# tkkim-robot/safe_control

Hardware: AMD Instinct MI355X
Metric: QP solves/sec (batched agents) (higher is better)
Workload: dtype f64; 1 GPU; 4096-agent batch DynamicUnicycle2D CBF-QP, 8 obstacles each (BASELINE configs[1]); agents_per_gpu=4096, obstacles=8, storage=f32, arithmetic=f64, launch=hipGraph

## Files before the change

### safe_control_amd/csrc/cbf_qp_kernel.hpp

```cpp
#pragma once
#include <hip/hip_runtime.h>

#include <utility>

#include <cstdlib>

#include "sc_qp2.hpp"
#include "sc_group.hpp"

namespace sc {

#ifndef SC_COOP_MAX_AGENTS
#define SC_COOP_MAX_AGENTS 32768
#endif

static inline long long sc_coop_max_agents() {
    static const long long v = [] { const char* e = getenv("SC_COOP_MAX_AGENTS"); return e ? atoll(e) : (long long)SC_COOP_MAX_AGENTS; }();
    return v;
}
static inline bool sc_two_pass() {
    static const bool v = [] { const char* e = getenv("SC_CBFQP_TWO_PASS"); return !(e && e[0] == '0'); }();
    return v;
}
static inline bool sc_force_lds_kernel() {
    static const bool v = [] { const char* e = getenv("SC_FORCE_LDS_KERNEL"); return e && e[0] == '1'; }();
    return v;
}

using as1_void = const __attribute__((address_space(1))) void;
using as3_void = __attribute__((address_space(3))) void;

template <typename TIO, int MODEL>
struct StateRow { TIO v[MODEL == SC_MODEL_QUAD2D ? 5 : 4]; };

template <typename TIO, int MODEL>
__device__ __forceinline__ StateRow<TIO, MODEL> load_state(const TIO* __restrict__ X, long long agent) {
    StateRow<TIO, MODEL> s;
    if constexpr (MODEL == SC_MODEL_QUAD2D) {
        const TIO* r = X + agent * 6;
#pragma unroll
        for (int i = 0; i < 5; ++i) s.v[i] = r[i];
    } else {
        const TIO* r = X + agent * 4;
#pragma unroll
        for (int i = 0; i < 4; ++i) s.v[i] = r[i];
    }
    return s;
}

template <typename TIO, typename TC, int MODEL>
__device__ __forceinline__ Agent<TC> to_agent(const StateRow<TIO, MODEL>& s) {
    if constexpr (MODEL == SC_MODEL_QUAD2D) return make_agent_m<TC, MODEL>(TC(s.v[0]), TC(s.v[1]), TC(s.v[2]), TC(s.v[3]), TC(s.v[4]));
    else return make_agent_m<TC, MODEL>(TC(s.v[0]), TC(s.v[1]), TC(s.v[2]), TC(s.v[3]));
}

template <typename TIO, typename TC, int MODEL>
__device__ __forceinline__ Agent<TC> load_agent(const TIO* __restrict__ X, long long agent) {
    return to_agent<TIO, TC, MODEL>(load_state<TIO, MODEL>(X, agent));
}

template <typename T>
__device__ __forceinline__ void fetch_arg_now(const T& v) { asm volatile("" ::"s"(v)); }

template <typename TIO> struct vec2;
template <> struct vec2<float> { using type = float2; };
template <> struct vec2<double> { using type = double2; };

__device__ __forceinline__ void wave_dma16(const unsigned char* __restrict__ src, unsigned char* lds,
                                           unsigned bytes, int lane) {
    const unsigned n16 = bytes >> 4;
    for (unsigned base = 0; base < n16; base += 64) {
        const unsigned idx = base + lane;
        if (idx < n16) {
            __builtin_amdgcn_global_load_lds((as1_void*)(src + (size_t)idx * 16),
                                             (as3_void*)(lds + (size_t)base * 16), 16, 0, 0);
        }
    }
}

template <typename TIO> struct vec4io;
template <> struct vec4io<float> { using type = float4; static constexpr int N = 4; };
template <> struct vec4io<double> { using type = double2; static constexpr int N = 2; };

#define SC_STATUS_PENDING (-1)
template <typename TIO, typename TC, int KMAX, int MODEL, int PASS = 0>
__global__ __launch_bounds__(256) void cbfqp_reg_kernel(const TIO* __restrict__ obs, const TIO* __restrict__ X,
                                                        const TIO* __restrict__ u_ref, const int* __restrict__ n_obs,
                                                        const long long B, const int K, const int obs_shared,
                                                        TIO* __restrict__ u_out, int* __restrict__ status_out,
                                                        TIO* __restrict__ h_out, const CbfConsts<TC> k) {
    const long long agent = (long long)blockIdx.x * blockDim.x + threadIdx.x;
    const bool active = agent < B;
    const long long ag_i = active ? agent : 0;
    using V2 = typename vec2<TIO>::type;
    using V4 = typename vec4io<TIO>::type;
    constexpr int VN = vec4io<TIO>::N;
    if constexpr (PASS == 2) {
        const bool pending = active && status_out[ag_i] == SC_STATUS_PENDING;
        if (__builtin_amdgcn_ballot_w64(pending) == 0ull) return;
    }

    TIO flat[KMAX * 7];
    const TIO* src = obs + (obs_shared ? 0 : (size_t)ag_i * K * 7);
    if (K == KMAX && ((KMAX * 7) % VN == 0) && ((reinterpret_cast<uintptr_t>(obs) & 15u) == 0) &&
        ((KMAX * 7 * sizeof(TIO)) % 16 == 0)) {
        const V4* s4 = reinterpret_cast<const V4*>(src);
#pragma unroll
        for (int e = 0; e < KMAX * 7 / VN; ++e) {
            const V4 q = s4[e];
            if constexpr (VN == 4) {
                flat[e * 4 + 0] = q.x; flat[e * 4 + 1] = q.y; flat[e * 4 + 2] = q.z; flat[e * 4 + 3] = q.w;
            } else {
                flat[e * 2 + 0] = q.x; flat[e * 2 + 1] = q.y;
            }
        }
    } else {
#pragma unroll
        for (int r = 0; r < KMAX; ++r) {
#pragma unroll
            for (int f = 0; f < 7; ++f) flat[r * 7 + f] = (r < K) ? src[r * 7 + f] : TIO(0);
        }
    }
    const V2 ur = reinterpret_cast<const V2*>(u_ref)[ag_i];
    const StateRow<TIO, MODEL> xs = load_state<TIO, MODEL>(X, ag_i);
    int nk = K;
    if (n_obs) nk = n_obs[ag_i];
    nk = nk < 0 ? 0 : (nk > K ? K : nk);
    if constexpr (PASS == 1) {
        bool other = false;
#pragma unroll
        for (int r = 0; r < KMAX; ++r) other |= (r < nk) && (flat[r * 7 + 6] != TIO(0));
        if (__builtin_amdgcn_ballot_w64(other && active) != 0ull) {
            if (active) status_out[agent] = SC_STATUS_PENDING;
            return;
        }
    }
    const TC ur0 = TC(ur.x), ur1 = TC(ur.y);
    const Agent<TC> ag = to_agent<TIO, TC, MODEL>(xs);

    TC n0[KMAX], n1[KMAX], c[KMAX];
    TIO hv[KMAX];
    bool bad_obs = false;
    TC poison = TC(0);
#pragma unroll
    for (int r = 0; r < KMAX; ++r) {
        TC o[7];
#pragma unroll
        for (int f = 0; f < 7; ++f) o[f] = TC(flat[r * 7 + f]);
        TC h, a0, a1, cc;
        const bool ok = cbf_row<TC, MODEL, true, PASS == 1>(ag, o, k, a0, a1, cc, h);
        const bool used = r < nk;
        bad_obs |= used && !ok;
        a0 = used ? a0 : TC(0); a1 = used ? a1 : TC(0); cc = used ? cc : TC(0);
        normalise_row(a0, a1, cc, poison);
        n0[r] = a0; n1[r] = a1; c[r] = cc;
        hv[r] = used ? TIO(h) : TIO(0);
    }

    TC u0, u1;
    int st = qp2_solve<TC, KMAX>(n0, n1, c, K, ur0, ur1, poison, k, u0, u1);
    if (bad_obs) st = SC_STATUS_BAD_OBSTACLE;
    if (st != SC_STATUS_OPTIMAL) { u0 = num<TC>::nan(); u1 = num<TC>::nan(); }
    if (active) {
        V2 uo; uo.x = TIO(u0); uo.y = TIO(u1);
        reinterpret_cast<V2*>(u_out)[agent] = uo;
        status_out[agent] = st;
        if (h_out) {
            TIO* hp = h_out + agent * K;
            if (K == KMAX && (KMAX % VN == 0) && ((reinterpret_cast<uintptr_t>(h_out) & 15u) == 0)) {
                V4* h4 = reinterpret_cast<V4*>(hp);
#pragma unroll
                for (int e = 0; e < KMAX / VN; ++e) {
                    V4 q;
                    if constexpr (VN == 4) { q.x = hv[e * 4]; q.y = hv[e * 4 + 1]; q.z = hv[e * 4 + 2]; q.w = hv[e * 4 + 3]; }
                    else { q.x = hv[e * 2]; q.y = hv[e * 2 + 1]; }
                    h4[e] = q;
                }
            } else {
#pragma unroll
                for (int r = 0; r < KMAX; ++r) if (r < K) hp[r] = hv[r];
            }
        }
    }
}

template <typename TIO, typename TC, int G, int MODEL>
#ifndef SC_COOP_WAVES
#define SC_COOP_WAVES 1
#endif
__global__ __launch_bounds__(64 * SC_COOP_WAVES) void cbfqp_coop_kernel(const TIO* __restrict__ obs, const TIO* __restrict__ X,
                                                        const TIO* __restrict__ u_ref, const int* __restrict__ n_obs,
                                                        const long long B, const int K, const int obs_shared,
                                                        TIO* __restrict__ u_out, int* __restrict__ status_out,
                                                        TIO* __restrict__ h_out, const CbfConsts<TC> k) {
#ifdef SC_EXP_EMPTY
    return;
#endif
    constexpr int APW = 64 / G;
    const int lane = threadIdx.x & 63;
    const int sub = lane & (G - 1);
    const long long agent = ((long long)blockIdx.x * SC_COOP_WAVES + (threadIdx.x >> 6)) * APW + lane / G;
    const bool active = agent < B;
    const long long ag_i = active ? agent : 0;
    using V2 = typename vec2<TIO>::type;
#ifdef SC_EXP_ARGS
    if (active && sub == 0)
        status_out[agent] = (int)((reinterpret_cast<uintptr_t>(obs) ^ reinterpret_cast<uintptr_t>(X) ^ reinterpret_cast<uintptr_t>(u_ref) ^
                                   reinterpret_cast<uintptr_t>(n_obs) ^ reinterpret_cast<uintptr_t>(u_out) ^ reinterpret_cast<uintptr_t>(h_out)) >> 4) + K + obs_shared;
    return;
#endif

    TIO orow[7];
    const bool has_row = sub < K;
    const TIO* src = obs + (obs_shared ? 0 : (size_t)ag_i * K * 7) + (has_row ? sub * 7 : 0);
#pragma unroll
    for (int f = 0; f < 7; ++f) orow[f] = src[f];
    const V2 ur = reinterpret_cast<const V2*>(u_ref)[ag_i];
    const StateRow<TIO, MODEL> xs = load_state<TIO, MODEL>(X, ag_i);
    int nk = K;
    if (n_obs) nk = n_obs[ag_i];
    nk = nk < 0 ? 0 : (nk > K ? K : nk);
    fetch_arg_now(status_out); fetch_arg_now(h_out);
    fetch_arg_now(k.R); fetch_arg_now(k.g1); fetch_arg_now(k.g2);
    fetch_arg_now(k.lo0); fetch_arg_now(k.hi0); fetch_arg_now(k.lo1); fetch_arg_now(k.hi1); fetch_arg_now(k.hard);
#ifdef SC_EXP_LOADS
    if (active) {
        if (sub == 0) {
            V2 uo; uo.x = ur.x + xs.v[0] + xs.v[1]; uo.y = ur.y + xs.v[2] + xs.v[3];
            reinterpret_cast<V2*>(u_out)[agent] = uo;
            status_out[agent] = nk;
        }
        if (h_out && has_row) h_out[agent * K + sub] = orow[0] + orow[1] + orow[2] + orow[3] + orow[4] + orow[5] + orow[6];
    }
    return;
#endif
    const TC ur0 = TC(ur.x), ur1 = TC(ur.y);
    const Agent<TC> ag = to_agent<TIO, TC, MODEL>(xs);

    TC o[7];
#pragma unroll
    for (int f = 0; f < 7; ++f) o[f] = TC(orow[f]);
    TC h, a0, a1, cc;
#ifndef SC_EXP_NOROW
    const bool ok = cbf_row<TC, MODEL, false>(ag, o, k, a0, a1, cc, h);
#else
    const bool ok = true; a0 = o[0] - ag.x; a1 = o[1] - ag.y; cc = o[2]; h = o[3];
#endif
    const bool used = sub < nk;
    const bool bad_mine = used && !ok;
    a0 = used ? a0 : TC(0); a1 = used ? a1 : TC(0); cc = used ? cc : TC(0);
    if (active && h_out && has_row) h_out[agent * K + sub] = used ? TIO(h) : TIO(0);
    TC poison = TC(0);
    normalise_row(a0, a1, cc, poison);

    QpState<TC> S;
    qp_begin(S, ur0, ur1, k);
#ifndef SC_EXP_NOWALK
#ifndef SC_COOP_OLD_WALK
    if constexpr (G == 8) coop_solve_all8<TC>(S, K, sub, lane, a0, a1, cc, k);
    else if constexpr (G == 16) coop_solve_all16<TC>(S, K, sub, lane, a0, a1, cc, k);
    else
#endif
    coop_walk_violated<TC, G>(S, K, sub, lane, a0, a1, cc, k);
#endif
    qp_finish_box(S, k);
    TC worst = qp_row_margin(num<TC>::inf(), a0, a1, cc, S.u0, S.u1, poison);
    const bool nan_mine = !(poison == poison);
    worst = nan_mine ? -num<TC>::inf() : worst;
    if constexpr (G == 8) worst = min8_raw(worst);
    else if constexpr (G == 16) worst = min16_raw(worst);
    else worst = group_min<TC, G>(worst);
    const unsigned long long bad_mask = __builtin_amdgcn_ballot_w64(bad_mine);
    const bool bad_any = ((bad_mask >> (lane & ~(G - 1))) & (G == 64 ? ~0ull : ((1ull << G) - 1ull))) != 0ull;
    int st = qp_status(S, worst, TC(0), k);
    if (bad_any) st = SC_STATUS_BAD_OBSTACLE;
    TC u0 = S.u0, u1 = S.u1;
    if (st != SC_STATUS_OPTIMAL) { u0 = num<TC>::nan(); u1 = num<TC>::nan(); }
    if (active) {
        if (sub == 0) {
            V2 uo; uo.x = TIO(u0); uo.y = TIO(u1);
            reinterpret_cast<V2*>(u_out)[agent] = uo;
            status_out[agent] = st;
        }
    }
}

template <typename TIO, typename TC, int G, int MODEL>
static hipError_t launch_coop(const sc_cbfqp_params& p, long long B, int K, const void* X, const void* u_ref,
                              const void* obs, const int* n_obs, void* u_out, int* status, void* h_out,
                              hipStream_t stream) {
    constexpr int APW = 64 / G;
    const unsigned nblk = (unsigned)((B + APW * SC_COOP_WAVES - 1) / (APW * SC_COOP_WAVES));
    const CbfConsts<TC> k = make_consts<TC>(p);
    hipLaunchKernelGGL((cbfqp_coop_kernel<TIO, TC, G, MODEL>), dim3(nblk), dim3(64 * SC_COOP_WAVES), 0, stream,
                       (const TIO*)obs, (const TIO*)X, (const TIO*)u_ref, n_obs, B, K, (int)p.obs_shared,
                       (TIO*)u_out, status, (TIO*)h_out, k);
    return hipGetLastError();
}

template <typename TIO, typename TC, int KMAX, int MODEL>
__global__ __launch_bounds__(64) void cbfqp_kernel(const TIO* __restrict__ obs, const TIO* __restrict__ X,
                                                   const TIO* __restrict__ u_ref, const int* __restrict__ n_obs,
                                                   const long long B, const int K, const int obs_shared,
                                                   TIO* __restrict__ u_out, int* __restrict__ status_out,
                                                   TIO* __restrict__ h_out, const CbfConsts<TC> k) {
    extern __shared__ __attribute__((aligned(16))) unsigned char smem[];
    TIO* lobs = reinterpret_cast<TIO*>(smem);

    const int lane = threadIdx.x;
    const long long first = (long long)blockIdx.x * 64;
    const long long agent = first + lane;
    const int nag = (int)((B - first) < 64 ? (B - first) : 64);
    const bool active = lane < nag;
    const int row_elems = K * 7;

    if (obs_shared) {
        for (int e = lane; e < row_elems; e += 64) lobs[e] = obs[e];
    } else {
        const TIO* src = obs + (size_t)first * row_elems;
        const unsigned bytes = (unsigned)nag * row_elems * sizeof(TIO);
        if ((bytes & 15u) == 0 && ((reinterpret_cast<uintptr_t>(src) & 15u) == 0)) {
            wave_dma16(reinterpret_cast<const unsigned char*>(src), smem, bytes, lane);
        } else {
            const int total = nag * row_elems;
            for (int e = lane; e < total; e += 64) lobs[e] = src[e];
        }
    }

    using V2 = typename vec2<TIO>::type;
    const long long ag_i = active ? agent : 0;
    const V2 ur = reinterpret_cast<const V2*>(u_ref)[ag_i];
    const StateRow<TIO, MODEL> xs = load_state<TIO, MODEL>(X, ag_i);
    int nk = K;
    if (n_obs) nk = n_obs[ag_i];
    nk = !active ? K : (nk < 0 ? 0 : (nk > K ? K : nk));
    const TC ur0 = active ? TC(ur.x) : TC(0), ur1 = active ? TC(ur.y) : TC(0);
    const Agent<TC> ag = to_agent<TIO, TC, MODEL>(xs);

    asm volatile("s_waitcnt vmcnt(0)" ::: "memory");
    __syncthreads();

    const size_t stage_bytes = ((obs_shared ? (size_t)row_elems : (size_t)64 * row_elems) * sizeof(TIO) + 15) & ~(size_t)15;
    TC* rows = reinterpret_cast<TC*>(smem + stage_bytes);
    TIO* hl = reinterpret_cast<TIO*>(rows + (size_t)K * 3 * 64);
    const TIO* mine = lobs + (obs_shared ? 0 : lane * row_elems);
    int period = 32;
    while (((K * (32 / period)) & 31) != 0 && period > 1) period >>= 1;
    const int rot = obs_shared ? 0 : (lane / period) % K;
    bool bad_obs = false;
    TC poison = TC(0);
#pragma nounroll
    for (int r = 0; r < K; ++r) {
        int ro = r + rot;
        ro = ro >= K ? ro - K : ro;
        TC o[7];
#pragma unroll
        for (int f = 0; f < 7; ++f) o[f] = TC(mine[ro * 7 + f]);
        TC h, a0, a1, cc;
        const bool ok = cbf_row<TC, MODEL>(ag, o, k, a0, a1, cc, h);
        const bool used = ro < nk;
        bad_obs |= used && !ok;
        a0 = used ? a0 : TC(0); a1 = used ? a1 : TC(0); cc = used ? cc : TC(0);
        normalise_row(a0, a1, cc, poison);
        rows[(ro * 3 + 0) * 64 + lane] = a0;
        rows[(ro * 3 + 1) * 64 + lane] = a1;
        rows[(ro * 3 + 2) * 64 + lane] = cc;
        if constexpr (KMAX > 0) {
            hl[ro * 64 + lane] = used ? TIO(h) : TIO(0);
        } else {
            if (active && h_out) h_out[agent * K + ro] = used ? TIO(h) : TIO(0);
        }
    }

    TC u0, u1;
    int st;
    if constexpr (KMAX > 0) {
        TC n0[KMAX], n1[KMAX], c[KMAX];
#pragma unroll
        for (int j = 0; j < KMAX; ++j) {
            const bool in = j < K;
            n0[j] = in ? rows[(j * 3 + 0) * 64 + lane] : TC(0);
            n1[j] = in ? rows[(j * 3 + 1) * 64 + lane] : TC(0);
            c[j] = in ? rows[(j * 3 + 2) * 64 + lane] : TC(0);
        }
        st = qp2_solve<TC, KMAX>(n0, n1, c, K, ur0, ur1, poison, k, u0, u1);
    } else {
        st = qp2_solve_lds<TC>(rows, lane, K, ur0, ur1, poison, k, u0, u1);
    }

    if (bad_obs) st = SC_STATUS_BAD_OBSTACLE;
    if (st != SC_STATUS_OPTIMAL) { u0 = num<TC>::nan(); u1 = num<TC>::nan(); }

    if (active) {
        V2 uo; uo.x = TIO(u0); uo.y = TIO(u1);
        reinterpret_cast<V2*>(u_out)[agent] = uo;
        status_out[agent] = st;
        if constexpr (KMAX > 0) {
            if (h_out) {
                TIO* hp = h_out + agent * K;
                if (K == KMAX) {
                    TIO hv[KMAX];
#pragma unroll
                    for (int r = 0; r < KMAX; ++r) hv[r] = hl[r * 64 + lane];
#pragma unroll
                    for (int r = 0; r < KMAX; ++r) hp[r] = hv[r];
                } else {
                    for (int r = 0; r < K; ++r) hp[r] = hl[r * 64 + lane];
                }
            }
        }
    }
}

template <typename TIO, typename TC, int KMAX, int MODEL>
static hipError_t launch_one(const sc_cbfqp_params& p, long long B, int K, const void* X, const void* u_ref,
                             const void* obs, const int* n_obs, void* u_out, int* status, void* h_out,
                             hipStream_t stream) {
    if constexpr (KMAX > 0) {
        if (B <= sc_coop_max_agents())
            return launch_coop<TIO, TC, 8, MODEL>(p, B, K, X, u_ref, obs, n_obs, u_out, status, h_out, stream);
        const unsigned threads = 256;
        const unsigned nblk = (unsigned)((B + threads - 1) / threads);
        const CbfConsts<TC> k = make_consts<TC>(p);
        if constexpr (MODEL == SC_MODEL_DYNAMIC_UNICYCLE2D && sizeof(TC) == 8) {
            if (sc_two_pass() && B >= (1 << 18)) {
                hipLaunchKernelGGL((cbfqp_reg_kernel<TIO, TC, KMAX, MODEL, 1>), dim3(nblk), dim3(threads), 0, stream,
                                   (const TIO*)obs, (const TIO*)X, (const TIO*)u_ref, n_obs, B, K, (int)p.obs_shared,
                                   (TIO*)u_out, status, (TIO*)h_out, k);
                hipError_t e = hipGetLastError();
                if (e != hipSuccess) return e;
                hipLaunchKernelGGL((cbfqp_reg_kernel<TIO, TC, KMAX, MODEL, 2>), dim3(nblk), dim3(threads), 0, stream,
                                   (const TIO*)obs, (const TIO*)X, (const TIO*)u_ref, n_obs, B, K, (int)p.obs_shared,
                                   (TIO*)u_out, status, (TIO*)h_out, k);
                return hipGetLastError();
            }
        }
        hipLaunchKernelGGL((cbfqp_reg_kernel<TIO, TC, KMAX, MODEL>), dim3(nblk), dim3(threads), 0, stream,
                           (const TIO*)obs, (const TIO*)X, (const TIO*)u_ref, n_obs, B, K, (int)p.obs_shared,
                           (TIO*)u_out, status, (TIO*)h_out, k);
        return hipGetLastError();
    } else {
    if (!sc_force_lds_kernel()) {
        if (K <= 16) return launch_coop<TIO, TC, 16, MODEL>(p, B, K, X, u_ref, obs, n_obs, u_out, status, h_out, stream);
        return launch_coop<TIO, TC, 32, MODEL>(p, B, K, X, u_ref, obs, n_obs, u_out, status, h_out, stream);
    }
    const unsigned blocks = (unsigned)((B + 63) / 64);
    const CbfConsts<TC> k = make_consts<TC>(p);
    size_t lds = (p.obs_shared ? (size_t)K * 7 : (size_t)64 * K * 7) * sizeof(TIO);
    lds = ((lds + 15) & ~(size_t)15) + (size_t)K * 3 * 64 * sizeof(TC) + (KMAX > 0 ? (size_t)K * 64 * sizeof(TIO) : 0);
    auto kern = cbfqp_kernel<TIO, TC, KMAX, MODEL>;
    if (lds > 64 * 1024) {
        static bool raised = false;
        if (!raised) {
            hipError_t e = hipFuncSetAttribute(reinterpret_cast<const void*>(kern),
                                               hipFuncAttributeMaxDynamicSharedMemorySize, 160 * 1024);
            if (e != hipSuccess) return e;
            raised = true;
        }
    }
    hipLaunchKernelGGL(kern, dim3(blocks), dim3(64), lds, stream,
                       (const TIO*)obs, (const TIO*)X, (const TIO*)u_ref, n_obs, B, K, (int)p.obs_shared,
                       (TIO*)u_out, status, (TIO*)h_out, k);
    return hipGetLastError();
    }
}

template <typename TIO, typename TC, int MODEL>
static hipError_t launch_k(const sc_cbfqp_params& p, long long B, int K, const void* X, const void* u_ref,
                           const void* obs, const int* n_obs, void* u_out, int* status, void* h_out,
                           hipStream_t stream) {
#define SC_K(KM) return launch_one<TIO, TC, KM, MODEL>(p, B, K, X, u_ref, obs, n_obs, u_out, status, h_out, stream)
    if (K <= 4) SC_K(4);
    if (K <= 8) SC_K(8);
    SC_K(0);
#undef SC_K
}

template <typename TIO, typename TC>
static hipError_t launch_model(const sc_cbfqp_params& p, long long B, int K, const void* X, const void* u_ref,
                               const void* obs, const int* n_obs, void* u_out, int* status, void* h_out,
                               hipStream_t stream) {
    switch (p.model_id) {
        case SC_MODEL_DYNAMIC_UNICYCLE2D:
            return launch_k<TIO, TC, SC_MODEL_DYNAMIC_UNICYCLE2D>(p, B, K, X, u_ref, obs, n_obs, u_out, status, h_out, stream);
        case SC_MODEL_KINEMATIC_BICYCLE2D:
            return launch_k<TIO, TC, SC_MODEL_KINEMATIC_BICYCLE2D>(p, B, K, X, u_ref, obs, n_obs, u_out, status, h_out, stream);
        case SC_MODEL_KINEMATIC_BICYCLE2D_C3BF:
            return launch_k<TIO, TC, SC_MODEL_KINEMATIC_BICYCLE2D_C3BF>(p, B, K, X, u_ref, obs, n_obs, u_out, status, h_out, stream);
        case SC_MODEL_SINGLE_INTEGRATOR2D:
            return launch_k<TIO, TC, SC_MODEL_SINGLE_INTEGRATOR2D>(p, B, K, X, u_ref, obs, n_obs, u_out, status, h_out, stream);
        case SC_MODEL_DOUBLE_INTEGRATOR2D:
            return launch_k<TIO, TC, SC_MODEL_DOUBLE_INTEGRATOR2D>(p, B, K, X, u_ref, obs, n_obs, u_out, status, h_out, stream);
        case SC_MODEL_QUAD2D:
            return launch_k<TIO, TC, SC_MODEL_QUAD2D>(p, B, K, X, u_ref, obs, n_obs, u_out, status, h_out, stream);
        case SC_MODEL_UNICYCLE2D:
            return launch_k<TIO, TC, SC_MODEL_UNICYCLE2D>(p, B, K, X, u_ref, obs, n_obs, u_out, status, h_out, stream);
        default:
            return launch_k<TIO, TC, SC_MODEL_KINEMATIC_BICYCLE2D_DPCBF>(p, B, K, X, u_ref, obs, n_obs, u_out, status, h_out, stream);
    }
}

}
```

### safe_control_amd/csrc/sc_group.hpp

```cpp
#pragma once
#include <hip/hip_runtime.h>

#include <utility>

#include "sc_qp2.hpp"

namespace sc {

template <int CTRL>
__device__ __forceinline__ float dpp_mov(float v) {
    return __int_as_float(__builtin_amdgcn_update_dpp(0, __float_as_int(v), CTRL, 0xf, 0xf, true));
}
template <int CTRL>
__device__ __forceinline__ double dpp_mov(double v) {
    const int lo = __builtin_amdgcn_update_dpp(0, __double2loint(v), CTRL, 0xf, 0xf, true);
    const int hi = __builtin_amdgcn_update_dpp(0, __double2hiint(v), CTRL, 0xf, 0xf, true);
    return __hiloint2double(hi, lo);
}
template <typename T, int G, int I>
__device__ __forceinline__ T group_bcast(T v, int sub) {
    if constexpr (G == 8) {
        const T q = dpp_mov<(I & 3) * 0x55>(v);
        const T m = dpp_mov<0x141>(q);
        return ((sub >> 2) == (I >> 2)) ? q : m;
    } else {
        return __shfl(v, I, G);
    }
}
template <typename T, int G>
__device__ __forceinline__ T group_max(T v) {
    if constexpr (G == 8) {
        v = fmax_(v, dpp_mov<0xB1>(v)); v = fmax_(v, dpp_mov<0x4E>(v)); v = fmax_(v, dpp_mov<0x141>(v));
    } else {
#pragma unroll
        for (int o = 1; o < G; o <<= 1) v = fmax_(v, __shfl_xor(v, o));
    }
    return v;
}
template <typename T, int G>
__device__ __forceinline__ T group_min(T v) {
    if constexpr (G == 8) {
        v = fmin_(v, dpp_mov<0xB1>(v)); v = fmin_(v, dpp_mov<0x4E>(v)); v = fmin_(v, dpp_mov<0x141>(v));
    } else {
#pragma unroll
        for (int o = 1; o < G; o <<= 1) v = fmin_(v, __shfl_xor(v, o));
    }
    return v;
}

template <typename TC, int G, int I>
__device__ __forceinline__ void coop_step(QpState<TC>& S, int K, int sub, TC a0, TC a1, TC cc, const CbfConsts<TC>& k) {
    if (I >= K) return;
    const TC bi0 = group_bcast<TC, G, I>(a0, sub), bi1 = group_bcast<TC, G, I>(a1, sub), bic = group_bcast<TC, G, I>(cc, sub);
    LineQP<TC> L;
    const bool viol = qp_row_violated(S, bi0, bi1, bic, L, k);
    if (__builtin_amdgcn_ballot_w64(viol) == 0) return;
    clip_box(L, k);
    if (sub < I) clip_row(L, a0, a1, cc);
    L.lo = group_max<TC, G>(L.lo);
    L.hi = group_min<TC, G>(L.hi);
    qp_row_commit(S, L, viol);
}
template <typename TC, int G, int... Is>
__device__ __forceinline__ void coop_walk(QpState<TC>& S, int K, int sub, TC a0, TC a1, TC cc, const CbfConsts<TC>& k,
                                          std::integer_sequence<int, Is...>) {
    (coop_step<TC, G, Is>(S, K, sub, a0, a1, cc, k), ...);
}

template <typename TC, int G>
__device__ __forceinline__ void coop_walk_violated(QpState<TC>& S, int K, int sub, int lane, TC a0, TC a1, TC cc,
                                                   const CbfConsts<TC>& k) {
    const int gbase = lane & ~(G - 1);
    const unsigned long long grp = (G == 64 ? ~0ull : ((1ull << G) - 1ull)) << gbase;
    const bool testable = (sub < K) && !((a0 == TC(0)) && (a1 == TC(0)));
    int last = -1;
#ifndef SC_EXP_MAXIT
#define SC_EXP_MAXIT G
#endif
    for (int it = 0; it < SC_EXP_MAXIT; ++it) {
        const TC s = a0 * S.u0 + (a1 * S.u1 + cc);
        const bool v = testable && (sub > last) && (s < TC(0));
        const unsigned long long m = __builtin_amdgcn_ballot_w64(v);
        if (m == 0ull) break;
        const unsigned long long mg = m & grp;
        const bool has = mg != 0ull;
        const int istar = has ? (__builtin_ctzll(mg) - gbase) : 0;
        const TC bi0 = __shfl(a0, istar, G), bi1 = __shfl(a1, istar, G), bic = __shfl(cc, istar, G);
        LineQP<TC> L;
        const bool viol = qp_row_violated(S, bi0, bi1, bic, L, k) && has;
        clip_box(L, k);
        if (sub < istar) clip_row(L, a0, a1, cc);
        L.lo = group_max<TC, G>(L.lo);
        L.hi = group_min<TC, G>(L.hi);
        qp_row_commit(S, L, viol);
        last = has ? istar : K;
    }
}

template <typename T, int X>
__device__ __forceinline__ T group_xor8(T v, T mirrored) {
    if constexpr (X == 1) return dpp_mov<0xB1>(v);
    else if constexpr (X == 2) return dpp_mov<0x4E>(v);
    else if constexpr (X == 3) return dpp_mov<0x1B>(v);
    else if constexpr (X == 4) return dpp_mov<0x1B>(mirrored);
    else if constexpr (X == 5) return dpp_mov<0x4E>(mirrored);
    else if constexpr (X == 6) return dpp_mov<0xB1>(mirrored);
    else return mirrored;
}
__device__ __forceinline__ float min_raw(float a, float b) { float r; asm("v_min_f32 %0, %1, %2" : "=v"(r) : "v"(a), "v"(b)); return r; }
__device__ __forceinline__ float max_raw(float a, float b) { float r; asm("v_max_f32 %0, %1, %2" : "=v"(r) : "v"(a), "v"(b)); return r; }
__device__ __forceinline__ double min_raw(double a, double b) { double r; asm("v_min_f64 %0, %1, %2" : "=v"(r) : "v"(a), "v"(b)); return r; }
__device__ __forceinline__ double max_raw(double a, double b) { double r; asm("v_max_f64 %0, %1, %2" : "=v"(r) : "v"(a), "v"(b)); return r; }
__device__ __forceinline__ float max_neg_raw(float a, float b) { float r; asm("v_max_f32 %0, %1, -%2" : "=v"(r) : "v"(a), "v"(b)); return r; }
__device__ __forceinline__ double max_neg_raw(double a, double b) { double r; asm("v_max_f64 %0, %1, -%2" : "=v"(r) : "v"(a), "v"(b)); return r; }
__device__ __forceinline__ float max_abs_one_raw(float a) { float r; asm("v_max_f32 %0, |%1|, 1.0" : "=v"(r) : "v"(a)); return r; }
__device__ __forceinline__ double max_abs_one_raw(double a) { double r; asm("v_max_f64 %0, |%1|, 1.0" : "=v"(r) : "v"(a)); return r; }
__device__ __forceinline__ float keep_or_nan(bool keep, float v) { return keep ? v : __int_as_float(0x7fc00000); }
__device__ __forceinline__ double keep_or_nan(bool keep, double v) {
    return __hiloint2double(keep ? __double2hiint(v) : 0x7ff80000, __double2loint(v));
}
template <typename T>
__device__ __forceinline__ T min8_raw(T v) {
    v = min_raw(v, dpp_mov<0xB1>(v)); v = min_raw(v, dpp_mov<0x4E>(v)); v = min_raw(v, dpp_mov<0x141>(v));
    return v;
}
template <typename T>
__device__ __forceinline__ T min16_raw(T v) { v = min8_raw(v); return min_raw(v, dpp_mov<0x140>(v)); }
template <int CTRL>
__device__ __forceinline__ int or_dpp(int v) { return v | __builtin_amdgcn_update_dpp(0, v, CTRL, 0xf, 0xf, true); }
template <int G>
__device__ __forceinline__ int group_or_bits(int v) {
    v = or_dpp<0xB1>(v); v = or_dpp<0x4E>(v); v = or_dpp<0x141>(v);
    if constexpr (G == 16) v = or_dpp<0x140>(v);
    return v;
}
template <int G>
__device__ __forceinline__ float group_pick(bool mine, float v) { return __int_as_float(group_or_bits<G>(mine ? __float_as_int(v) : 0)); }
template <int G>
__device__ __forceinline__ double group_pick(bool mine, double v) {
    const int lo = group_or_bits<G>(mine ? __double2loint(v) : 0), hi = group_or_bits<G>(mine ? __double2hiint(v) : 0);
    return __hiloint2double(hi, lo);
}

template <typename T>
__device__ __forceinline__ void clip_row_coop(LineQP<T>& L, bool& dead, T g0, T g1, T gc) {
    const T a = g0 * L.d0 + g1 * L.d1;
    const T r = g0 * L.p0 + (g1 * L.p1 + gc);
    const bool pos = a > num<T>::eps_par();
    const bool neg = !(a >= -num<T>::eps_par());
    const bool par_viol = r < -num<T>::tol_feas() * max_abs_one_raw(gc);
    const T q = r * rcp_(fabs_(a));
    dead |= !pos && !neg && par_viol;
    L.lo = max_neg_raw(L.lo, keep_or_nan(pos, q));
    L.hi = min_raw(L.hi, keep_or_nan(neg, q));
}

template <int G>
__device__ __forceinline__ bool group_first(unsigned long long m, int lane, int sub, bool& has) {
    const unsigned bits = (unsigned)(m >> (lane & ~(G - 1))) & ((1u << G) - 1u);
    has = bits != 0u;
    return sub == __builtin_ctz(bits | (1u << G));
}

template <typename TC, int... Xs>
__device__ __forceinline__ void clip_partners8(LineQP<TC>& L, bool& dead, TC a0, TC a1, TC cc, std::integer_sequence<int, Xs...>) {
    const TC m0 = dpp_mov<0x141>(a0), m1 = dpp_mov<0x141>(a1), mc = dpp_mov<0x141>(cc);
    (clip_row_coop(L, dead, group_xor8<TC, Xs + 1>(a0, m0), group_xor8<TC, Xs + 1>(a1, m1), group_xor8<TC, Xs + 1>(cc, mc)), ...);
}
template <typename TC, int G>
__device__ __forceinline__ void coop_pick_winner(QpState<TC>& S, const LineQP<TC>& L, bool ok, int sub, int lane) {
    const TC inf = num<TC>::inf();
    TC t = fmin_(fmax_(TC(0), L.lo), L.hi);
    const bool inverted = L.lo > L.hi;
    t = inverted ? TC(0.5) * (L.lo + L.hi) : t;
    const bool empty = L.lo > L.hi + num<TC>::tol_feas() * fmax_(TC(1), fmax_(fabs_(L.lo), fabs_(L.hi)));
    const TC v0 = L.p0 + t * L.d0, v1 = L.p1 + t * L.d1;
    const TC e0 = v0 - S.ur0, e1 = v1 - S.ur1;
    TC cost = e0 * e0 + e1 * e1;
    cost = (ok && !empty && (cost == cost)) ? cost : inf;
    TC best;
    if constexpr (G == 8) best = min8_raw(cost); else best = min16_raw(cost);
    bool has;
    const bool mine = group_first<G>(__builtin_amdgcn_ballot_w64((cost == best) && (best < inf)), lane, sub, has);
    const TC s0 = group_pick<G>(mine, v0), s1 = group_pick<G>(mine, v1);
    S.u0 = has ? s0 : S.u0;
    S.u1 = has ? s1 : S.u1;
}
template <typename TC>
__device__ __forceinline__ void coop_solve_all8(QpState<TC>& S, int K, int sub, int lane, TC a0, TC a1, TC cc,
                                                const CbfConsts<TC>& k) {
    const bool testable = (sub < K) && !((a0 == TC(0)) && (a1 == TC(0)));
    LineQP<TC> L;
    const bool viol = qp_row_violated(S, a0, a1, cc, L, k) && testable;
    if (__builtin_amdgcn_ballot_w64(viol) == 0ull) return;
    clip_box(L, k);
    bool dead = false;
    clip_partners8(L, dead, a0, a1, cc, std::make_integer_sequence<int, 7>{});
    coop_pick_winner<TC, 8>(S, L, viol && !dead, sub, lane);
}

template <typename TC, int... Rs>
__device__ __forceinline__ void clip_partners16(LineQP<TC>& L, bool& dead, TC a0, TC a1, TC cc, std::integer_sequence<int, Rs...>) {
    (clip_row_coop(L, dead, dpp_mov<0x121 + Rs>(a0), dpp_mov<0x121 + Rs>(a1), dpp_mov<0x121 + Rs>(cc)), ...);
}
template <typename TC>
__device__ __forceinline__ void coop_solve_all16(QpState<TC>& S, int K, int sub, int lane, TC a0, TC a1, TC cc,
                                                 const CbfConsts<TC>& k) {
    const bool testable = (sub < K) && !((a0 == TC(0)) && (a1 == TC(0)));
    LineQP<TC> L;
    const bool viol = qp_row_violated(S, a0, a1, cc, L, k) && testable;
    if (__builtin_amdgcn_ballot_w64(viol) == 0ull) return;
    clip_box(L, k);
    bool dead = false;
    clip_partners16(L, dead, a0, a1, cc, std::make_integer_sequence<int, 15>{});
    coop_pick_winner<TC, 16>(S, L, viol && !dead, sub, lane);
}

}
```

### safe_control_amd/csrc/sc_math.hpp

```cpp
#pragma once
#include <hip/hip_runtime.h>
#include <cmath>
#include <cstdint>

namespace sc {

template <typename T> struct num;
template <> struct num<float> {
    static __device__ __forceinline__ float inf() { return __builtin_huge_valf(); }
    static __device__ __forceinline__ float nan() { return __builtin_nanf(""); }
    static __device__ __forceinline__ float eps_par() { return 1e-5f; }
    static __device__ __forceinline__ float tol_feas() { return 1e-5f; }
};
template <> struct num<double> {
    static __device__ __forceinline__ double inf() { return __builtin_huge_val(); }
    static __device__ __forceinline__ double nan() { return __builtin_nan(""); }
    static __device__ __forceinline__ double eps_par() { return 1e-12; }
    static __device__ __forceinline__ double tol_feas() { return 1e-9; }
};

__device__ __forceinline__ void sincos_(float x, float* s, float* c) { sincosf(x, s, c); }
__device__ __forceinline__ void sincos_(double x, double* s, double* c) {
    if (!(fabs(x) < 1.0e5)) { sincos(x, s, c); return; }
    const double k = rint(x * 0.63661977236758138);
    double r = __builtin_fma(-k, 1.5707963267948966, x);
    r = __builtin_fma(-k, 6.123233995736766e-17, r);
    r = __builtin_fma(-k, -1.4973849048591698e-33, r);
    const double z = r * r;
    double ps = __builtin_fma(z, 1.58969099521155010221e-10, -2.50507602534068634195e-08);
    ps = __builtin_fma(z, ps, 2.75573137070700676789e-06);
    ps = __builtin_fma(z, ps, -1.98412698298579493134e-04);
    ps = __builtin_fma(z, ps, 8.33333333332248946124e-03);
    const double ks = __builtin_fma(z * r, __builtin_fma(z, ps, -1.66666666666666324348e-01), r);
    double pc = __builtin_fma(z, -1.13596475577881948265e-11, 2.08757232129817482790e-09);
    pc = __builtin_fma(z, pc, -2.75573143513906633035e-07);
    pc = __builtin_fma(z, pc, 2.48015872894767294178e-05);
    pc = __builtin_fma(z, pc, -1.38888888888741095749e-03);
    pc = __builtin_fma(z, pc, 4.16666666666666019037e-02);
    const double hz = 0.5 * z, w = 1.0 - hz;
    const double kc = w + (((1.0 - w) - hz) + z * (z * pc));
    const int n = (int)k & 3;
    const double sv = (n & 1) ? kc : ks, cv = (n & 1) ? ks : kc;
    *s = (n & 2) ? -sv : sv;
    *c = ((n + 1) & 2) ? -cv : cv;
}
__device__ __forceinline__ float sqrt_(float x) { return sqrtf(x); }
__device__ __forceinline__ double sqrt_(double x) { return sqrt(x); }
__device__ __forceinline__ float fabs_(float x) { return fabsf(x); }
__device__ __forceinline__ double fabs_(double x) { return fabs(x); }
__device__ __forceinline__ float fmax_(float a, float b) { return fmaxf(a, b); }
__device__ __forceinline__ double fmax_(double a, double b) { return fmax(a, b); }
__device__ __forceinline__ float fmin_(float a, float b) { return fminf(a, b); }
__device__ __forceinline__ double fmin_(double a, double b) { return fmin(a, b); }
__device__ __forceinline__ float pow_(float a, float b) { return powf(a, b); }
__device__ __forceinline__ double pow_(double a, double b) { return pow(a, b); }
__device__ __forceinline__ float rint_(float a) { return rintf(a); }
__device__ __forceinline__ double rint_(double a) { return rint(a); }
__device__ __forceinline__ float atan2_(float a, float b) { return atan2f(a, b); }
__device__ __forceinline__ double atan2_(double a, double b) { return atan2(a, b); }
__device__ __forceinline__ float floor_(float a) { return floorf(a); }
__device__ __forceinline__ double floor_(double a) { return floor(a); }
__device__ __forceinline__ bool finite_(float a) { return __builtin_isfinite(a); }
__device__ __forceinline__ bool finite_(double a) { return __builtin_isfinite(a); }

template <typename T>
__device__ __forceinline__ T powi_chain(T x, int n) {
    T r = T(1), b = x;
    while (n) {
        if (n & 1) r *= b;
        b *= b;
        n >>= 1;
    }
    return r;
}

__device__ __forceinline__ float fmod_(float a, float b) { return fmodf(a, b); }
__device__ __forceinline__ double fmod_(double a, double b) { return fmod(a, b); }

template <typename T>
__device__ __forceinline__ T pymod(T x, T m) {
    T r = fmod_(x, m);
    if (r < T(0)) r += m;
    return r;
}

template <typename T>
__device__ __forceinline__ T angle_normalize(T x) {
    const T pi = T(3.14159265358979323846);
    return pymod(x + pi, T(2) * pi) - pi;
}

}
```

Measured before the change: 1.484 billion solves/s.

## Add specialised coop8 DynamicUnicycle2D kernel with packed kernarg constants

```diff
diff --git a/safe_control_amd/csrc/cbf_qp_kernel.hpp b/safe_control_amd/csrc/cbf_qp_kernel.hpp
--- a/safe_control_amd/csrc/cbf_qp_kernel.hpp
+++ b/safe_control_amd/csrc/cbf_qp_kernel.hpp
@@ -285,12 +285,149 @@
     }
 }
 
+typedef double sc_d8 __attribute__((ext_vector_type(8)));
+struct Coop8Consts {
+    sc_d8 t0;
+    sc_d8 t1;
+    sc_d8 k0;
+    sc_d8 k1;
+    int hard;
+    unsigned B;
+};
+
+__device__ __forceinline__ void normalise_row_as_generic(double& n0, double& n1, double& c, double& poison) {
+    const double nn = __builtin_fma(n1, n1, n0 * n0);
+    poison += 0.0 * (nn + c);
+    const double inv = nn > 0.0 ? rsqrt_(nn) : 1.0;
+    n0 *= inv; n1 *= inv; c *= inv;
+}
+
+template <typename TIO, bool FULL, bool HAS_H>
+__global__ __launch_bounds__(64) void cbfqp_coop8_du_kernel(const TIO* __restrict__ obs, const TIO* __restrict__ X,
+                                                            const TIO* __restrict__ u_ref, TIO* __restrict__ u_out,
+                                                            TIO* __restrict__ h_out, int* __restrict__ status_out,
+                                                            const Coop8Consts c) {
+#ifdef SC_EXP_EMPTY
+    return;
+#endif
+    using TC = double;
+    using V2 = typename vec2<TIO>::type;
+    const unsigned lane = threadIdx.x;
+    const unsigned sub = lane & 7u;
+    const unsigned slot = blockIdx.x * 64u + lane;
+    const unsigned agent = slot >> 3;
+    bool active = true;
+    if constexpr (!FULL) active = agent < c.B;
+    const unsigned row_i = active ? slot : sub;
+    const unsigned ag_i = row_i >> 3;
+
+    struct { TIO v[7]; } orow;
+    __builtin_memcpy(&orow, obs + row_i * 7u, sizeof(orow));
+    const V2 ur = reinterpret_cast<const V2*>(u_ref)[ag_i];
+    const StateRow<TIO, SC_MODEL_DYNAMIC_UNICYCLE2D> xs = load_state<TIO, SC_MODEL_DYNAMIC_UNICYCLE2D>(X, ag_i);
+    fetch_arg_now(c.t0); fetch_arg_now(c.t1); fetch_arg_now(c.k0); fetch_arg_now(c.k1); fetch_arg_now(c.hard);
+
+    SinCosTab sc;
+    sc.two_over_pi = c.t0[0]; sc.pio2_1 = c.t0[1]; sc.pio2_2 = c.t0[2]; sc.pio2_3 = c.t0[3];
+    sc.s[0] = c.t0[4]; sc.s[1] = c.t0[5]; sc.s[2] = c.t0[6]; sc.s[3] = c.t0[7]; sc.s[4] = c.t1[0]; sc.s[5] = c.t1[1];
+#pragma unroll
+    for (int i = 0; i < 6; ++i) sc.c[i] = c.t1[2 + i];
+    CbfConsts<TC> k;
+    k.R = c.k0[0]; k.a1 = TC(0); k.a2 = TC(0); k.g1 = c.k0[1]; k.g2 = c.k0[2]; k.inv_dt = c.k0[3]; k.inv_dt2 = c.k0[4];
+    k.lo0 = c.k0[5]; k.hi0 = c.k0[6]; k.lo1 = c.k0[7]; k.hi1 = c.k1[0]; k.inv_Lr = TC(0); k.inv_mass = TC(1); k.hard = c.hard;
+    BoxTol<TC> bt;
+    bt.lo0 = c.k1[1]; bt.hi0 = c.k1[2]; bt.lo1 = c.k1[3]; bt.hi1 = c.k1[4];
+
+    const TC ur0 = TC(ur.x), ur1 = TC(ur.y);
+    Agent<TC> ag;
+    ag.x = TC(xs.v[0]); ag.y = TC(xs.v[1]); ag.th = TC(xs.v[2]); ag.v = TC(xs.v[3]);
+    sincos_tab(ag.th, sc, &ag.s, &ag.c);
+    ag.f0 = ag.v * ag.c;
+    ag.f1 = ag.v * ag.s;
+
+    TC o[7];
+#pragma unroll
+    for (int f = 0; f < 7; ++f) o[f] = TC(orow.v[f]);
+    TC h, a0, a1, cc;
+    const bool ok = cbf_row<TC, SC_MODEL_DYNAMIC_UNICYCLE2D, false>(ag, o, k, a0, a1, cc, h);
+    const bool bad_mine = !ok;
+    if constexpr (HAS_H) {
+        if (active) h_out[slot] = TIO(h);
+    }
+    TC poison = TC(0);
+    normalise_row_as_generic(a0, a1, cc, poison);
+
+    QpState<TC> S;
+    qp_begin(S, ur0, ur1, k);
+    coop_solve_all8_full<TC>(S, (int)sub, (int)lane, a0, a1, cc, k, bt);
+    qp_finish_box(S, k);
+    TC worst = qp_row_margin(num<TC>::inf(), a0, a1, cc, S.u0, S.u1, poison);
+    const bool nan_mine = !(poison == poison);
+    worst = nan_mine ? -num<TC>::inf() : worst;
+    worst = min8_raw(worst);
+    const unsigned long long bad_mask = __builtin_amdgcn_ballot_w64(bad_mine);
+    const bool bad_any = ((bad_mask >> (lane & ~7u)) & 0xffull) != 0ull;
+    int st = qp_status(S, worst, TC(0), k);
+    if (bad_any) st = SC_STATUS_BAD_OBSTACLE;
+    TC u0 = S.u0, u1 = S.u1;
+    if (st != SC_STATUS_OPTIMAL) { u0 = num<TC>::nan(); u1 = num<TC>::nan(); }
+    if (active && sub == 0) {
+        V2 uo; uo.x = TIO(u0); uo.y = TIO(u1);
+        reinterpret_cast<V2*>(u_out)[agent] = uo;
+        status_out[agent] = st;
+    }
+}
+
+#if defined(SC_EXP_GRID) && !defined(SC_EXP_EMPTY)
+#error "SC_EXP_GRID needs SC_EXP_EMPTY: a kernel with a body would run past the batch"
+#endif
+static inline unsigned coop_grid(unsigned nblk) {
+#ifdef SC_EXP_GRID
+    return SC_EXP_GRID;
+#else
+    return nblk;
+#endif
+}
+
+static inline bool sc_cbfqp_generic() {
+    static const bool v = [] { const char* e = getenv("SC_CBFQP_GENERIC"); return e && e[0] == '1'; }();
+    return v;
+}
+
+template <typename TIO>
+static hipError_t launch_coop8_du(const sc_cbfqp_params& p, long long B, const void* X, const void* u_ref, const void* obs,
+                                  void* u_out, int* status, void* h_out, hipStream_t stream) {
+    const CbfConsts<double> k = make_consts<double>(p);
+    const BoxTol<double> bt = box_tol(k);
+    const SinCosTab t = make_sincos_tab();
+    Coop8Consts c;
+    c.t0 = sc_d8{t.two_over_pi, t.pio2_1, t.pio2_2, t.pio2_3, t.s[0], t.s[1], t.s[2], t.s[3]};
+    c.t1 = sc_d8{t.s[4], t.s[5], t.c[0], t.c[1], t.c[2], t.c[3], t.c[4], t.c[5]};
+    c.k0 = sc_d8{k.R, k.g1, k.g2, k.inv_dt, k.inv_dt2, k.lo0, k.hi0, k.lo1};
+    c.k1 = sc_d8{k.hi1, bt.lo0, bt.hi0, bt.lo1, bt.hi1, 0.0, 0.0, 0.0};
+    c.hard = k.hard;
+    c.B = (unsigned)B;
+    const dim3 grid(coop_grid((unsigned)((B + 7) / 8))), block(64);
+#define SC_GO(FULL, HAS_H)                                                                                             \
+    hipLaunchKernelGGL((cbfqp_coop8_du_kernel<TIO, FULL, HAS_H>), grid, block, 0, stream, (const TIO*)obs, (const TIO*)X, \
+                       (const TIO*)u_ref, (TIO*)u_out, (TIO*)h_out, status, c)
+    if (B % 8 == 0) { if (h_out) SC_GO(true, true); else SC_GO(true, false); }
+    else { if (h_out) SC_GO(false, true); else SC_GO(false, false); }
+#undef SC_GO
+    return hipGetLastError();
+}
+
 template <typename TIO, typename TC, int G, int MODEL>
 static hipError_t launch_coop(const sc_cbfqp_params& p, long long B, int K, const void* X, const void* u_ref,
                               const void* obs, const int* n_obs, void* u_out, int* status, void* h_out,
                               hipStream_t stream) {
+    if constexpr (G == 8 && MODEL == SC_MODEL_DYNAMIC_UNICYCLE2D && sizeof(TC) == 8 && SC_COOP_WAVES == 1) {
+        if (K == 8 && n_obs == nullptr && p.obs_shared == 0 && B >= 1 && B <= sc_coop_max_agents() &&
+            B * 8 * 7 * (long long)sizeof(TIO) <= 0x7fffffffLL && !sc_cbfqp_generic())
+            return launch_coop8_du<TIO>(p, B, X, u_ref, obs, u_out, status, h_out, stream);
+    }
     constexpr int APW = 64 / G;
-    const unsigned nblk = (unsigned)((B + APW * SC_COOP_WAVES - 1) / (APW * SC_COOP_WAVES));
+    const unsigned nblk = coop_grid((unsigned)((B + APW * SC_COOP_WAVES - 1) / (APW * SC_COOP_WAVES)));
     const CbfConsts<TC> k = make_consts<TC>(p);
     hipLaunchKernelGGL((cbfqp_coop_kernel<TIO, TC, G, MODEL>), dim3(nblk), dim3(64 * SC_COOP_WAVES), 0, stream,
                        (const TIO*)obs, (const TIO*)X, (const TIO*)u_ref, n_obs, B, K, (int)p.obs_shared,
diff --git a/safe_control_amd/csrc/sc_group.hpp b/safe_control_amd/csrc/sc_group.hpp
--- a/safe_control_amd/csrc/sc_group.hpp
+++ b/safe_control_amd/csrc/sc_group.hpp
@@ -199,6 +199,50 @@
     coop_pick_winner<TC, 8>(S, L, viol && !dead, sub, lane);
 }
 
+template <typename T>
+struct BoxTol { T lo0, hi0, lo1, hi1; };
+template <typename T>
+__host__ __device__ inline BoxTol<T> box_tol(const CbfConsts<T>& k) {
+    const T tol = sizeof(T) == 8 ? T(1e-9) : T(1e-5f);
+    BoxTol<T> b;
+    b.lo0 = k.lo0 - tol; b.hi0 = k.hi0 + tol; b.lo1 = k.lo1 - tol; b.hi1 = k.hi1 + tol;
+    return b;
+}
+template <typename T>
+__device__ __forceinline__ void clip_box_tol(LineQP<T>& L, const CbfConsts<T>& k, const BoxTol<T>& bt) {
+    const T inf = num<T>::inf();
+    {
+        const T r = rcp_(L.d0);
+        const T t1 = (k.lo0 - L.p0) * r, t2 = (k.hi0 - L.p0) * r;
+        const bool flat = L.d0 == T(0);
+        const bool inside = (L.p0 >= bt.lo0) && (L.p0 <= bt.hi0);
+        const T lo = flat ? (inside ? -inf : inf) : fmin_(t1, t2);
+        const T hi = flat ? inf : fmax_(t1, t2);
+        L.lo = lo; L.hi = hi;
+    }
+    {
+        const T r = rcp_(L.d1);
+        const T t1 = (k.lo1 - L.p1) * r, t2 = (k.hi1 - L.p1) * r;
+        const bool flat = L.d1 == T(0);
+        const bool inside = (L.p1 >= bt.lo1) && (L.p1 <= bt.hi1);
+        const T lo = flat ? (inside ? -inf : inf) : fmin_(t1, t2);
+        const T hi = flat ? inf : fmax_(t1, t2);
+        L.lo = fmax_(L.lo, lo); L.hi = fmin_(L.hi, hi);
+    }
+}
+template <typename TC>
+__device__ __forceinline__ void coop_solve_all8_full(QpState<TC>& S, int sub, int lane, TC a0, TC a1, TC cc,
+                                                     const CbfConsts<TC>& k, const BoxTol<TC>& bt) {
+    const bool testable = !((a0 == TC(0)) && (a1 == TC(0)));
+    LineQP<TC> L;
+    const bool viol = qp_row_violated(S, a0, a1, cc, L, k) && testable;
+    if (__builtin_amdgcn_ballot_w64(viol) == 0ull) return;
+    clip_box_tol(L, k, bt);
+    bool dead = false;
+    clip_partners8(L, dead, a0, a1, cc, std::make_integer_sequence<int, 7>{});
+    coop_pick_winner<TC, 8>(S, L, viol && !dead, sub, lane);
+}
+
 template <typename TC, int... Rs>
 __device__ __forceinline__ void clip_partners16(LineQP<TC>& L, bool& dead, TC a0, TC a1, TC cc, std::integer_sequence<int, Rs...>) {
     (clip_row_coop(L, dead, dpp_mov<0x121 + Rs>(a0), dpp_mov<0x121 + Rs>(a1), dpp_mov<0x121 + Rs>(cc)), ...);
diff --git a/safe_control_amd/csrc/sc_math.hpp b/safe_control_amd/csrc/sc_math.hpp
--- a/safe_control_amd/csrc/sc_math.hpp
+++ b/safe_control_amd/csrc/sc_math.hpp
@@ -37,6 +37,45 @@
     pc = __builtin_fma(z, pc, 2.48015872894767294178e-05);
     pc = __builtin_fma(z, pc, -1.38888888888741095749e-03);
     pc = __builtin_fma(z, pc, 4.16666666666666019037e-02);
+    const double hz = 0.5 * z, w = 1.0 - hz;
+    const double kc = w + (((1.0 - w) - hz) + z * (z * pc));
+    const int n = (int)k & 3;
+    const double sv = (n & 1) ? kc : ks, cv = (n & 1) ? ks : kc;
+    *s = (n & 2) ? -sv : sv;
+    *c = ((n + 1) & 2) ? -cv : cv;
+}
+struct SinCosTab {
+    double two_over_pi, pio2_1, pio2_2, pio2_3;
+    double s[6];
+    double c[6];
+};
+__host__ __device__ inline SinCosTab make_sincos_tab() {
+    SinCosTab t;
+    t.two_over_pi = 0.63661977236758138;
+    t.pio2_1 = 1.5707963267948966; t.pio2_2 = 6.123233995736766e-17; t.pio2_3 = -1.4973849048591698e-33;
+    t.s[0] = 1.58969099521155010221e-10; t.s[1] = -2.50507602534068634195e-08; t.s[2] = 2.75573137070700676789e-06;
+    t.s[3] = -1.98412698298579493134e-04; t.s[4] = 8.33333333332248946124e-03; t.s[5] = -1.66666666666666324348e-01;
+    t.c[0] = -1.13596475577881948265e-11; t.c[1] = 2.08757232129817482790e-09; t.c[2] = -2.75573143513906633035e-07;
+    t.c[3] = 2.48015872894767294178e-05; t.c[4] = -1.38888888888741095749e-03; t.c[5] = 4.16666666666666019037e-02;
+    return t;
+}
+__device__ __forceinline__ void sincos_tab(double x, const SinCosTab& t, double* s, double* c) {
+    if (!(fabs(x) < 1.0e5)) { sincos(x, s, c); return; }
+    const double k = rint(x * t.two_over_pi);
+    double r = __builtin_fma(-k, t.pio2_1, x);
+    r = __builtin_fma(-k, t.pio2_2, r);
+    r = __builtin_fma(-k, t.pio2_3, r);
+    const double z = r * r;
+    double ps = __builtin_fma(z, t.s[0], t.s[1]);
+    ps = __builtin_fma(z, ps, t.s[2]);
+    ps = __builtin_fma(z, ps, t.s[3]);
+    ps = __builtin_fma(z, ps, t.s[4]);
+    const double ks = __builtin_fma(z * r, __builtin_fma(z, ps, t.s[5]), r);
+    double pc = __builtin_fma(z, t.c[0], t.c[1]);
+    pc = __builtin_fma(z, pc, t.c[2]);
+    pc = __builtin_fma(z, pc, t.c[3]);
+    pc = __builtin_fma(z, pc, t.c[4]);
+    pc = __builtin_fma(z, pc, t.c[5]);
     const double hz = 0.5 * z, w = 1.0 - hz;
     const double kc = w + (((1.0 - w) - hz) + z * (z * pc));
     const int n = (int)k & 3;
```

New measurement: 1.573 billion solves/s, median of 6. 6.0% higher.
